# angela000/DQNFlappyBird

Hardware: NVIDIA B200
Metric: env frames/sec (step+render+preproc) (higher is better)
Workload: dtype u8

## Files before the change

dqnflappybird_b200/_lib.py:

```python
from __future__ import annotations

import ctypes as C
import glob
import os
import subprocess

_PKG = os.path.dirname(os.path.abspath(__file__))
_CSRC = os.path.join(_PKG, "csrc")
SO_PATH = os.path.join(_PKG, "libflappy_b200.so")

NVCC_FLAGS = [
    "-gencode", "arch=compute_100a,code=sm_100a", "-lineinfo", "-O3", "-std=c++17",
    "-Xcompiler", "-fPIC", "-shared",
]


class FlappyError(RuntimeError):
    pass


def sources():
    return sorted(glob.glob(os.path.join(_CSRC, "*.cu")))


# ... 61 lines not shown
                ("eps", C.c_float), ("grad_scale", C.c_float), ("beta1_power", C.c_float), ("beta2_power", C.c_float)]


_SIGNATURES = {
    "fb_last_error": ([], C.c_char_p),
    "fb_version": ([], C.c_int),
    "fb_assets_load": ([C.c_char_p, C.c_size_t], C.c_int),
    "fb_resize_tables": ([_i32p], C.c_int),
    "fb_env_create": ([C.c_int, C.c_uint64, C.c_uint64, C.POINTER(C.c_void_p)], C.c_int),
    "fb_env_destroy": ([_vp], C.c_int),
    "fb_env_num_envs": ([_vp], C.c_int),
    "fb_env_set_gap_replay": ([_vp, _u8p, C.c_int], C.c_int),
    "fb_env_reset": ([_vp, _vp], C.c_int),
    "fb_env_step": ([_vp, C.c_int, _u8p, _u8p, C.c_int, C.c_int, _f32p, _u8p, _i32p, _vp], C.c_int),
    "fb_env_draw": ([_vp, _u8p, C.c_int, C.c_int, _vp], C.c_int),
    "fb_env_step_random": ([_vp, C.c_int, C.c_uint64, C.c_uint32, C.c_uint32, _u8p, _u8p, C.c_int, C.c_int,
                            _f32p, _u8p, _i32p, _vp], C.c_int),
    "fb_env_step_host": ([_vp, _u8p, _u8p, C.c_int, C.c_int, _f32p, _u8p, _i32p, _vp], C.c_int),
    "fb_env_step_host_submit": ([_vp, _u8p, _u8p, C.c_int, C.c_int, _f32p, _u8p, _i32p, _vp], C.c_int),
    "fb_env_step_host_wait": ([_vp], C.c_int),
    "fb_env_check": ([_vp, _vp], C.c_int),
    "fb_env_export_state": ([_vp, _i32p, _vp], C.c_int),
    "fb_env_import_state": ([_vp, _i32p, _vp], C.c_int),
    "fb_env_obs_exact": ([_vp, _u8p, _vp], C.c_int),
    "fb_render_full": ([_vp, C.c_int, C.c_int, _u8p, _vp], C.c_int),
    "fb_log_episodes": ([_u8p, _i32p, C.c_int, C.c_int, C.c_int, _i32p, _i32p, C.c_int, _vp], C.c_int),
    "fb_qnet_create": ([C.c_int, C.c_int, C.c_int, C.POINTER(C.c_void_p)], C.c_int),
    "fb_qnet_destroy": ([_vp], C.c_int),
    "fb_qnet_set_precision": ([_vp, C.c_int], C.c_int),
    "fb_qnet_get_precision": ([_vp], C.c_int),
    "fb_qnet_invalidate": ([_vp], C.c_int),
    "fb_qnet_set_per_broadcast": ([_vp, C.c_int], C.c_int),
    "fb_debug_poison_packed": ([_vp, C.c_int, _vp], C.c_int),
    "fb_debug_write_probe": ([_vp, C.c_int, C.c_longlong, C.c_int, C.c_int, _vp], C.c_int),
    "fb_qnet_use_graphs": ([_vp, C.c_int], C.c_int),
    "fb_qnet_set_conv1_mode": ([_vp, C.c_int], C.c_int),
    "fb_qnet_set_fused_backward": ([_vp, C.c_int], C.c_int),
    "fb_qnet_param_count": ([_vp], C.c_int),
    "fb_qnet_layout": ([_vp, _i32p], C.c_int),
    "fb_qnet_forward": ([_vp, _f32p, _u8p, C.c_longlong, _i32p, C.c_int, _f32p, _vp], C.c_int),
    "fb_qnet_act": ([_vp, _f32p, _u8p, C.c_longlong, _i32p, C.c_int, C.c_double, C.c_uint64, C.c_uint64, _vp, _f32p, _u8p, _vp], C.c_int),
    "fb_qnet_adam": ([_vp, _f32p, _f32p, _f32p, _f32p, C.c_float, C.c_float, C.c_float, C.c_float, C.c_float, _vp], C.c_int),
    "fb_qnet_step": ([_vp, _vp, _vp], C.c_int),
    "fb_qnet_sync_target": ([_vp, _f32p, _f32p, _vp], C.c_int),
    "fb_noisy_layout": ([_vp, _i32p], C.c_int),
    "fb_noisy_draw": ([_vp, C.c_uint64, C.c_int, C.c_uint64, _f32p, _vp], C.c_int),
    "fb_noisy_weights": ([_vp, _f32p, _f32p, _f32p, _f32p, _vp], C.c_int),
    "fb_qnet_noisy_adam": ([_vp, _f32p, _f32p, _f32p, _f32p, _f32p, _f32p, _f32p, _f32p, C.c_float, C.c_float, C.c_float, C.c_float,
                            C.c_float, _vp], C.c_int),
    "fb_debug_struct_layout": ([C.c_int, _i32p, C.c_int], C.c_int),
    "fb_debug_step_sampling_layout": ([_i32p, C.c_int], C.c_int),
    "fb_dist_debug_stamps": ([_vp, _vp], C.c_int),
    "fb_dist_create": ([C.c_int, C.c_int, C.c_longlong, C.POINTER(C.c_void_p)], C.c_int),
    "fb_dist_destroy": ([_vp], C.c_int),
    "fb_dist_handle_bytes": ([], C.c_int),
    "fb_dist_set_two_shot": ([_vp, C.c_int], C.c_int),
    "fb_dist_debug_mask": ([_vp, C.c_int], C.c_int),
    "fb_dist_handles": ([_vp, C.c_char_p], C.c_int),
    "fb_dist_connect": ([_vp, C.c_char_p], C.c_int),
    "fb_dist_connect_local": ([_vp, C.c_int, _vp], C.c_int),
    "fb_dist_grads": ([_vp, C.c_int, C.POINTER(C.c_void_p)], C.c_int),
    "fb_dist_parity": ([_vp], C.c_int),
    "fb_dist_advance": ([_vp], C.c_int),
    "fb_qnet_attach_exchange": ([_vp, _vp], C.c_int),
    "fb_dist_adam": ([_vp, _vp, _f32p, _f32p, _f32p, C.c_float, C.c_float, C.c_float, C.c_float, C.c_float, _f32p, C.c_int, _vp], C.c_int),
    "fb_replay_create": ([C.c_int, C.c_int, C.c_int, C.c_int, C.c_int, C.POINTER(C.c_void_p)], C.c_int),
    "fb_replay_destroy": ([_vp], C.c_int),
# ... 61 lines not shown
```

dqnflappybird_b200/csrc/fb_debug.cu:

```cuda
#include <stddef.h>
#include <string.h>

#include "fb_env_logic.cuh"

extern "C" int fb_debug_host_step(int32_t *state16, int action, const uint8_t *gaps, int gaps_len, uint64_t seed,
                                  uint64_t env_id, float *reward, uint8_t *terminal, int32_t *score) {
    const ExactTables *ex = fb_host_exact_tables();
    if (!ex) { fb_set_error("fb_debug_host_step: load the assets first"); return FB_ERR_ASSETS; }
    FB_REQUIRE(state16 && reward && terminal && score, "fb_debug_host_step: NULL argument");
    if (action != 0 && action != 1) { fb_set_error("Multiple input actions!"); return FB_ERR_ACTION; }
    EnvState s;
    memset(&s, 0, sizeof(s));
    if (!ints_to_state(state16, s)) { fb_set_error("fb_debug_host_step: state outside the reachable range"); return FB_ERR_STATE; }
    GapSource g{gaps, gaps_len, seed, env_id};
    env_step(s, action, g, ex, *reward, *terminal, *score);
    state_to_ints(s, state16);
    return FB_OK;
}

extern "C" int fb_debug_host_reset(int32_t *state16, const uint8_t *gaps, int gaps_len, uint64_t seed, uint64_t env_id) {
    FB_REQUIRE(state16 != nullptr, "fb_debug_host_reset: NULL argument");
    EnvState s;
    memset(&s, 0, sizeof(s));
    GapSource g{gaps, gaps_len, seed, env_id};
// ... 35 lines not shown
    memset(&s, 0, sizeof(s));
    if (!ints_to_state(state16, s)) return -1;
    return (make_draw_list(s).np_mixed & 16) ? 1 : 0;
}

#define FB_OFF(S, f) (int32_t) offsetof(S, f)
extern "C" int fb_debug_struct_layout(int which, int32_t *out, int capacity) {
    typedef fb_step_sampling S;
    typedef fb_qnet_step_args A;
    const int32_t sampling[] = {(int32_t)sizeof(S), FB_OFF(S, replay), FB_OFF(S, ring_dev), FB_OFF(S, act_dev), FB_OFF(S, rew_dev),
                                FB_OFF(S, term_dev), FB_OFF(S, t), FB_OFF(S, batch), FB_OFF(S, setsize), FB_OFF(S, seed),
                                FB_OFF(S, idx_out_dev), FB_OFF(S, frames_out_dev), FB_OFF(S, act_out_dev), FB_OFF(S, rew_out_dev),
                                FB_OFF(S, term_out_dev), FB_OFF(S, env_out_dev), FB_OFF(S, k_out_dev), FB_OFF(S, prioritized),
                                FB_OFF(S, per_mode), FB_OFF(S, beta), FB_OFF(S, tree_idx_out_dev), FB_OFF(S, is_weights_out_dev),
                                FB_OFF(S, prio_out_dev), FB_OFF(S, is_weights_f32_out_dev), FB_OFF(S, n_step), FB_OFF(S, ret_out_dev),
                                FB_OFF(S, disc_out_dev)};
    const int32_t step[] = {(int32_t)sizeof(A), FB_OFF(A, variant), FB_OFF(A, loss_sum), FB_OFF(A, batch), FB_OFF(A, global_batch),
                            FB_OFF(A, gamma), FB_OFF(A, params_dev), FB_OFF(A, target_params_dev), FB_OFF(A, sampling),
                            FB_OFF(A, frames_dev), FB_OFF(A, sample_stride), FB_OFF(A, chan_off_s), FB_OFF(A, chan_off_next),
                            FB_OFF(A, actions_dev), FB_OFF(A, rewards_dev), FB_OFF(A, terminals_dev), FB_OFF(A, is_weights_dev),
                            FB_OFF(A, grads_dev), FB_OFF(A, loss_out_dev), FB_OFF(A, abs_err_out_dev), FB_OFF(A, q_target_out_dev),
                            FB_OFF(A, m_dev), FB_OFF(A, v_dev), FB_OFF(A, lr), FB_OFF(A, beta1), FB_OFF(A, beta2), FB_OFF(A, eps),
                            FB_OFF(A, grad_scale), FB_OFF(A, beta1_power), FB_OFF(A, beta2_power)};
    FB_REQUIRE(which == 0 || which == 1, "fb_debug_struct_layout: which must be 0 (fb_step_sampling) or 1 (fb_qnet_step_args)");
    const int32_t *v = which == 0 ? sampling : step;
    const int n = which == 0 ? (int)(sizeof(sampling) / sizeof(sampling[0])) : (int)(sizeof(step) / sizeof(step[0]));
    FB_REQUIRE(out != nullptr && capacity >= n, "fb_debug_struct_layout: buffer too small");
    for (int i = 0; i < n; i++) out[i] = v[i];
    return n;
}
#undef FB_OFF
extern "C" int fb_debug_step_sampling_layout(int32_t *out, int capacity) { return fb_debug_struct_layout(0, out, capacity); }

__global__ void __launch_bounds__(256) write_probe_kernel(uint8_t *dst, int n_chunks, long long stride_bytes, int mode) {
    extern __shared__ __align__(128) uint8_t stage_all[];
    const int warp = threadIdx.x >> 5, lane = threadIdx.x & 31;
    uint8_t *stage = stage_all + warp * 6400;
    const long long W = (long long)gridDim.x * 8, w = (long long)blockIdx.x * 8 + warp;
    const int lo = (int)((long long)n_chunks * w / W), hi = (int)((long long)n_chunks * (w + 1) / W);
    if (mode == 1) {
        for (int i = lane; i < 400; i += 32) reinterpret_cast<uint4 *>(stage)[i] = make_uint4(i, lane, 0xFFFFFFFFu, 0);
        asm volatile("fence.proxy.async.shared::cta;" ::: "memory");
        __syncwarp();
    }
    for (int k = lo; k < hi; k++) {
        uint8_t *out = dst + (long long)k * stride_bytes;
        if (mode == 0) {
            const uint4 v = make_uint4(k, lane, 0xFFFFFFFFu, 0);
#pragma unroll
            for (int it = 0; it < 13; it++) { int c = lane + 32 * it; if (c < 400) __stcs(reinterpret_cast<uint4 *>(out) + c, v); }
        } else if (lane == 0) {
            asm volatile("cp.async.bulk.wait_group.read 0;" ::: "memory");
            asm volatile("cp.async.bulk.global.shared::cta.bulk_group [%0], [%1], 6400;" ::"l"(reinterpret_cast<uint64_t>(out)),
                         "r"((uint32_t)__cvta_generic_to_shared(stage)) : "memory");
            asm volatile("cp.async.bulk.commit_group;" ::: "memory");
        }
    }
    if (mode == 1 && lane == 0) asm volatile("cp.async.bulk.wait_group 0;" ::: "memory");
}

extern "C" int fb_debug_write_probe(uint8_t *dst_dev, int n_chunks, long long stride_bytes, int mode, int ctas, void *stream) {
    FB_REQUIRE(dst_dev && n_chunks > 0 && stride_bytes >= 6400 && (mode == 0 || mode == 1) && ctas > 0, "fb_debug_write_probe: bad argument");
    FB_CUDA_OK(cudaFuncSetAttribute(write_probe_kernel, cudaFuncAttributeMaxDynamicSharedMemorySize, 8 * 6400));
    write_probe_kernel<<<ctas, 256, 8 * 6400, (cudaStream_t)stream>>>(dst_dev, n_chunks, stride_bytes, mode);
    FB_CUDA_OK(cudaGetLastError());
    return FB_OK;
}
```

dqnflappybird_b200/csrc/fb_env.cu:

```cuda
#include <stdlib.h>

#include <new>

#include "fb_env_logic.cuh"

struct fb_env {
    int n;
    uint64_t seed, first_id;
    EnvState *state;
    const uint8_t *gaps;
    int gaps_len;
    int *err_flag;
    uint8_t *stage_act[2];
    float *stage_rew[2];
    uint8_t *stage_term[2];
    int32_t *stage_score[2];
    cudaStream_t s_in, s_out;
    cudaEvent_t ev_in[2], ev_step[2], ev_out[2];
    unsigned long long submitted, waited;
    int num_sms;
    int step_slots;
};

struct StepArgs {
    EnvState *state;
    int n;
    uint64_t seed, first_id;
    const uint8_t *gaps;
    int gaps_len;
    const uint8_t *actions;
    uint64_t act_seed;
    uint32_t first_step, flap_threshold;
    uint8_t *actions_out;
    uint8_t *ring;
    int ring_len, ring_slot;
    float *reward;
    uint8_t *terminal;
    int32_t *score;
    int n_steps;
    int draw_only;
    int *err_flag;
    const ObsTables *obs_tab;
    const ExactTables *ex;
};

__device__ __forceinline__ uint32_t expand4(uint32_t nib) {
    return ((nib * 0x00204081u) & 0x01010101u) * 255u;
}

struct RowConst { int sx[3], tab[3]; };

struct __align__(16) DrawWords {
    int px[3];
    int flags;
    int goff[3];
    int bird;
};
__device__ __forceinline__ DrawWords to_words(const ObsTables &T, const DrawList &d) {
    DrawWords w;
    const int np = d.np_mixed & 15;
#pragma unroll
    for (int k = 0; k < 3; k++) { w.px[k] = k < np ? (int)d.px[k] : 9999; w.goff[k] = (int)d.gap[k] * 8; }
    w.flags = ((d.np_mixed & 16) ? 1 : 0) | ((int)T.birdJ0[d.y] << 1) | ((int)d.y << 8) | ((int)d.pidx << 20) | (np << 24);
    w.bird = ((int)d.pidx * (kMaxY + 1) + (int)d.y) * (kBirdRows + 3);
    return w;
}

constexpr int kChunks = kObs * 5;

__device__ __forceinline__ void render_env(const ObsTables &T, const uint2 *lut8, const ExactTables *ex, const DrawWords w,
                                           const RowConst &rc, unsigned short *m16, unsigned long long *fixrows, uint8_t *out, int lane) {
    const int j0 = (w.flags >> 1) & 127;
    const unsigned char *pipe_bytes = reinterpret_cast<const unsigned char *>(&T.pipeObs[0][0][0]);
    const unsigned char *bird_bytes = reinterpret_cast<const unsigned char *>(&T.birdObs[0][0][0]) + w.bird;
// ... 21 lines not shown
            int idx = q * 32 + lane, r = idx >> 3, j = j0 + (idx & 7);
            int bit = 0;
            if (r < kBirdRows && j < kBaseJ) bit = exact_obs_bit(ex, d, 0, false, 16 + r, j);
            unsigned bal = __ballot_sync(0xFFFFFFFFu, bit);
            int rr = 4 * q + lane;
            if (lane < 4 && rr < kBirdRows) fixrows[rr] = obs_row_fix(fixrows[rr], (bal >> (8 * lane)) & 0xFFu, j0);
        }
        __syncwarp();
        if (lane >= 16 && lane < 16 + kBirdRows) m[0] = fixrows[lane - 16];
    }
#pragma unroll
    for (int it = 0; it < 3; it++) {
        const int i = lane + 32 * it;
        if (i < kObs) {
            unsigned short *row = m16 + 5 * i;
            row[0] = (unsigned short)m[it]; row[1] = (unsigned short)(m[it] >> 16);
            row[2] = (unsigned short)(m[it] >> 32); row[3] = (unsigned short)(m[it] >> 48);
        }
    }
    __syncwarp();
    const unsigned short *mine = m16 + lane;
    uint4 *dst = reinterpret_cast<uint4 *>(out) + lane;
#pragma unroll
    for (int it = 0; it < 13; it++) {
        if (it < 12 || lane < kChunks - 32 * 12) {
            const uint32_t bits = mine[32 * it];
            const uint2 a = lut8[bits & 255u], b = lut8[bits >> 8];
            __stcs(dst + 32 * it, make_uint4(a.x, a.y, b.x, b.y));
        }
    }
    __syncwarp();
}

constexpr int kStepThreads = 256, kStepWarps = kStepThreads / 32;

__global__ void __launch_bounds__(kStepThreads, 4) env_step_kernel(const StepArgs a) {
    extern __shared__ __align__(16) unsigned char t_raw[];
    ObsTables &T = *reinterpret_cast<ObsTables *>(t_raw);
    __shared__ __align__(16) HitTables H;
    __shared__ DrawWords dw[kStepWarps][32];
    __shared__ __align__(16) unsigned short m16[kStepWarps][kChunks + 8];
    __shared__ unsigned long long fixrows[kStepWarps][kBirdRows + 1];
    __shared__ uint2 lut8[256];
    const int tid = threadIdx.x, warp = tid >> 5, lane = tid & 31;
    asm volatile("griddepcontrol.launch_dependents;");
    lut8[tid] = make_uint2(expand4(tid & 15u), expand4(tid >> 4));

    {
        const uint4 *srcH = reinterpret_cast<const uint4 *>(a.ex);
        uint4 *dstH = reinterpret_cast<uint4 *>(&H);
        for (int k = tid; k < (int)(sizeof(HitTables) / 16); k += kStepThreads) dstH[k] = __ldg(srcH + k);
    }
    if (a.ring) {
        const uint4 *src = reinterpret_cast<const uint4 *>(a.obs_tab);
        uint4 *dstT = reinterpret_cast<uint4 *>(&T);
        for (int k = tid; k < (int)(sizeof(ObsTables) / 16); k += kStepThreads) dstT[k] = __ldg(src + k);
    }
    __syncthreads();
    asm volatile("griddepcontrol.wait;" ::: "memory");

    RowConst rc;
#pragma unroll
    for (int it = 0; it < 3; it++) {
        const int i = min(lane + 32 * it, kObs - 1);
        rc.sx[it] = T.sx[i]; rc.tab[it] = (i - 5 * ((i * 205) >> 10)) * 64;
    }
    for (int i = lane; i < kObs; i += 32) m16[warp][5 * i + 4] = 0xFFFFu;
    __syncwarp();
    const long long W = (long long)gridDim.x * kStepWarps, w = (long long)blockIdx.x * kStepWarps + warp;
    const int lo = (int)((long long)a.n * w / W), hi = (int)((long long)a.n * (w + 1) / W);
    for (int base = lo; base < hi; base += 32) {
        const int e_mine = base + lane;
        const bool have = e_mine < hi;
        const int n_here = min(32, hi - base);
        EnvState s;
        GapSource gs;
        if (have) {
            const uint4 *sp = reinterpret_cast<const uint4 *>(a.state + e_mine);
            uint4 v0 = sp[0], v1 = sp[1];
            *reinterpret_cast<uint4 *>(&s) = v0;
            *(reinterpret_cast<uint4 *>(&s) + 1) = v1;
            gs.script = a.gaps ? a.gaps + (size_t)e_mine * a.gaps_len : nullptr;
            gs.script_len = a.gaps_len;
            gs.seed = a.seed; gs.env_id = a.first_id + (uint64_t)e_mine;
        }
        for (int step = 0; step < a.n_steps; step++) {
            if (have && a.draw_only) dw[warp][lane] = to_words(T, make_draw_list(s));
            if (have && !a.draw_only) {
                int act;
                const size_t o = (size_t)step * a.n + e_mine;
                if (a.actions) {
                    act = a.actions[o];
                    if (act > 1) { atomicOr(a.err_flag, 1); act = 0; }
                } else {
                    act = stream_word(a.act_seed, 1u, gs.env_id, a.first_step + (uint32_t)step) < a.flap_threshold ? 1 : 0;
                    if (a.actions_out) a.actions_out[o] = (uint8_t)act;
                }
                float rew; uint8_t term; int32_t sc;
                env_step(s, act, gs, &H, rew, term, sc);
                if (a.reward) a.reward[o] = rew;
                if (a.terminal) a.terminal[o] = term;
                if (a.score) a.score[o] = sc;
                if (a.ring) dw[warp][lane] = to_words(T, make_draw_list(s));
            }
            if (a.ring) {
                const int slot = (a.ring_slot + step) % a.ring_len;
                __syncwarp();
                for (int e = 0; e < n_here; e++) {
                    uint8_t *out = a.ring + ((size_t)(base + e) * a.ring_len + slot) * (size_t)FB_FRAME_BYTES;
                    render_env(T, lut8, a.ex, dw[warp][e], rc, m16[warp], fixrows[warp], out, lane);
                }
                __syncwarp();
            }
        }
        if (have) {
            uint4 *sp = reinterpret_cast<uint4 *>(a.state + e_mine);
            sp[0] = *reinterpret_cast<uint4 *>(&s);
            sp[1] = *(reinterpret_cast<uint4 *>(&s) + 1);
        }
    }
}


__global__ void env_reset_kernel(EnvState *state, int n, uint64_t seed, uint64_t first_id, const uint8_t *gaps, int gaps_len) {
    int e = blockIdx.x * blockDim.x + threadIdx.x;
    if (e >= n) return;
    EnvState s;
    memset(&s, 0, sizeof(s));
    GapSource gs{gaps ? gaps + (size_t)e * gaps_len : nullptr, gaps_len, seed, first_id + (uint64_t)e};
    env_reset(s, gs);
    state[e] = s;
}

__global__ void env_export_kernel(const EnvState *state, int n, int32_t *out) {
    int e = blockIdx.x * blockDim.x + threadIdx.x;
    if (e >= n) return;
    EnvState s = state[e];
    state_to_ints(s, out + (size_t)e * FB_STATE_INTS);
}

__global__ void env_import_kernel(EnvState *state, int n, const int32_t *in, int *err_flag) {
    int e = blockIdx.x * blockDim.x + threadIdx.x;
    if (e >= n) return;
    EnvState s;
    if (!ints_to_state(in + (size_t)e * FB_STATE_INTS, s)) { atomicOr(err_flag, 2); return; }
    state[e] = s;
}

__global__ void env_obs_exact_kernel(const EnvState *state, int n, const ExactTables *ex, uint8_t *obs) {
    int e = blockIdx.x;
    if (e >= n) return;
    __shared__ DrawList d;
// ... 5 lines not shown
        obs[(size_t)e * FB_FRAME_BYTES + p] = exact_obs_bit(ex, d, basex, true, i, j) ? 255 : 0;
    }
}

__global__ void env_render_full_kernel(const EnvState *state, int first, int n, const ExactTables *ex, uint8_t *rgb) {
    int e = blockIdx.y;
    if (e >= n) return;
    __shared__ DrawList d;
    __shared__ int basex;
    if (threadIdx.x == 0) { EnvState s = state[first + e]; d = make_draw_list(s); basex = s.basex; }
    __syncthreads();
    int p = blockIdx.x * blockDim.x + threadIdx.x;
    if (p >= kScreenW * kScreenH) return;
    int X = p / kScreenH, Y = p - X * kScreenH;
    uint32_t c = scene_rgb(ex, d, basex, true, X, Y);
    uint8_t *o = rgb + ((size_t)e * kScreenW * kScreenH + p) * 3;
    o[0] = c & 255; o[1] = (c >> 8) & 255; o[2] = (c >> 16) & 255;
}


extern "C" int fb_env_create(int n_envs, uint64_t seed, uint64_t first_env_id, fb_env **out) {
    FB_REQUIRE(out != nullptr, "fb_env_create: out is NULL");
    FB_REQUIRE(n_envs > 0, "fb_env_create: n_envs must be positive");
    if (!fb_tables().loaded) { fb_set_error("fb_env_create: call fb_assets_load first"); return FB_ERR_ASSETS; }
    fb_env *e = new (std::nothrow) fb_env();
    FB_REQUIRE(e != nullptr, "fb_env_create: out of host memory");
    e->n = n_envs; e->seed = seed; e->first_id = first_env_id; e->gaps = nullptr; e->gaps_len = 0;
    int dev = 0;
    FB_CUDA_OK(cudaGetDevice(&dev));
    FB_CUDA_OK(cudaDeviceGetAttribute(&e->num_sms, cudaDevAttrMultiProcessorCount, dev));
    FB_CUDA_OK(cudaMalloc(&e->state, sizeof(EnvState) * (size_t)n_envs));
    FB_CUDA_OK(cudaMalloc(&e->err_flag, sizeof(int)));
    FB_CUDA_OK(cudaMemset(e->err_flag, 0, sizeof(int)));
    for (int k = 0; k < 2; k++) {
        FB_CUDA_OK(cudaMalloc(&e->stage_act[k], (size_t)n_envs));
        FB_CUDA_OK(cudaMalloc(&e->stage_rew[k], sizeof(float) * (size_t)n_envs));
        FB_CUDA_OK(cudaMalloc(&e->stage_term[k], (size_t)n_envs));
        FB_CUDA_OK(cudaMalloc(&e->stage_score[k], sizeof(int32_t) * (size_t)n_envs));
        FB_CUDA_OK(cudaEventCreateWithFlags(&e->ev_in[k], cudaEventDisableTiming));
        FB_CUDA_OK(cudaEventCreateWithFlags(&e->ev_step[k], cudaEventDisableTiming));
        FB_CUDA_OK(cudaEventCreateWithFlags(&e->ev_out[k], cudaEventDisableTiming));
    }
    FB_CUDA_OK(cudaStreamCreateWithFlags(&e->s_in, cudaStreamNonBlocking));
    FB_CUDA_OK(cudaStreamCreateWithFlags(&e->s_out, cudaStreamNonBlocking));
    e->submitted = e->waited = 0;
    e->step_slots = 0;
    *out = e;
    return fb_env_reset(e, nullptr);
}

extern "C" int fb_env_destroy(fb_env *e) {
    if (!e) return FB_OK;
    cudaFree(e->state); cudaFree(e->err_flag);
    for (int k = 0; k < 2; k++) {
        cudaFree(e->stage_act[k]); cudaFree(e->stage_rew[k]); cudaFree(e->stage_term[k]); cudaFree(e->stage_score[k]);
        if (e->ev_in[k]) cudaEventDestroy(e->ev_in[k]);
        if (e->ev_step[k]) cudaEventDestroy(e->ev_step[k]);
        if (e->ev_out[k]) cudaEventDestroy(e->ev_out[k]);
    }
    if (e->s_in) cudaStreamDestroy(e->s_in);
    if (e->s_out) cudaStreamDestroy(e->s_out);
    delete e;
    return FB_OK;
}

extern "C" int fb_env_num_envs(const fb_env *e) { return e ? e->n : 0; }

extern "C" int fb_env_set_gap_replay(fb_env *e, const uint8_t *gaps_dev, int per_env_len) {
    FB_REQUIRE(e != nullptr, "fb_env_set_gap_replay: env is NULL");
    FB_REQUIRE(gaps_dev == nullptr || per_env_len > 0, "fb_env_set_gap_replay: per_env_len must be positive");
    e->gaps = gaps_dev; e->gaps_len = gaps_dev ? per_env_len : 0;
    return FB_OK;
}

extern "C" int fb_env_reset(fb_env *e, void *stream) {
    FB_REQUIRE(e != nullptr, "fb_env_reset: env is NULL");
    env_reset_kernel<<<(e->n + 255) / 256, 256, 0, (cudaStream_t)stream>>>(e->state, e->n, e->seed, e->first_id, e->gaps, e->gaps_len);
    FB_CUDA_OK(cudaGetLastError());
    return FB_OK;
}

static int launch_step(fb_env *e, StepArgs &a, cudaStream_t st, bool early = true) {
    a.state = e->state; a.n = e->n; a.seed = e->seed; a.first_id = e->first_id;
    a.gaps = e->gaps; a.gaps_len = e->gaps_len; a.err_flag = e->err_flag;
    a.obs_tab = fb_tables().obs_dev; a.ex = fb_tables().exact_dev;
    if (e->step_slots == 0) {
        FB_CUDA_OK(cudaFuncSetAttribute(env_step_kernel, cudaFuncAttributeMaxDynamicSharedMemorySize, (int)sizeof(ObsTables)));
        int per_sm = 0;
        FB_CUDA_OK(cudaOccupancyMaxActiveBlocksPerMultiprocessor(&per_sm, env_step_kernel, kStepThreads, sizeof(ObsTables)));
        FB_REQUIRE(per_sm >= 1, "env_step_kernel does not fit an SM");
        e->step_slots = per_sm * e->num_sms;
    }
    static int oversub = 0;
    if (oversub == 0) { const char *v = getenv("FB_ENV_OVERSUB"); oversub = (v && v[0] >= '1' && v[0] <= '8') ? v[0] - '0' : 1; }
    long long warps = (long long)e->step_slots * kStepWarps * oversub;
    if (warps > e->n) warps = e->n;
    const int grid = (int)((warps + kStepWarps - 1) / kStepWarps);
    cudaLaunchConfig_t cfg{};
    cfg.gridDim = dim3(grid); cfg.blockDim = dim3(kStepThreads); cfg.dynamicSmemBytes = sizeof(ObsTables); cfg.stream = st;
    cudaLaunchAttribute at[1];
    at[0].id = cudaLaunchAttributeProgrammaticStreamSerialization;
    static int pdl = -1;
    if (pdl < 0) { const char *v = getenv("FB_ENV_PDL"); pdl = (v && v[0] == '0') ? 0 : 1; }
    at[0].val.programmaticStreamSerializationAllowed = pdl && early ? 1 : 0;
    cfg.attrs = at; cfg.numAttrs = 1;
    FB_CUDA_OK(cudaLaunchKernelEx(&cfg, env_step_kernel, (const StepArgs)a));
    return FB_OK;
}

static int check_ring(const fb_env *e, const uint8_t *ring, int ring_len, int ring_slot, int n_steps) {
    FB_REQUIRE(e != nullptr, "fb_env_step: env is NULL");
    FB_REQUIRE(n_steps > 0, "fb_env_step: n_steps must be positive");
    if (ring) {
        FB_REQUIRE(ring_len > 0 && ring_slot >= 0 && ring_slot < ring_len, "fb_env_step: ring_slot outside the ring");
        FB_REQUIRE((reinterpret_cast<uintptr_t>(ring) & 15) == 0, "fb_env_step: obs ring must be 16-byte aligned");
    }
    return FB_OK;
}

extern "C" int fb_env_step(fb_env *e, int n_steps, const uint8_t *actions_dev, uint8_t *obs_ring_dev, int ring_len,
                           int ring_slot, float *reward_dev, uint8_t *terminal_dev, int32_t *score_dev, void *stream) {
    int rc = check_ring(e, obs_ring_dev, ring_len, ring_slot, n_steps);
    if (rc) return rc;
    FB_REQUIRE(actions_dev != nullptr, "fb_env_step: actions_dev is NULL");
    StepArgs a{};
    a.actions = actions_dev; a.ring = obs_ring_dev; a.ring_len = ring_len; a.ring_slot = ring_slot;
    a.reward = reward_dev; a.terminal = terminal_dev; a.score = score_dev; a.n_steps = n_steps;
    return launch_step(e, a, (cudaStream_t)stream);
}

extern "C" int fb_env_draw(fb_env *e, uint8_t *obs_ring_dev, int ring_len, int ring_slot, void *stream) {
    int rc = check_ring(e, obs_ring_dev, ring_len, ring_slot, 1);
    if (rc) return rc;
    FB_REQUIRE(obs_ring_dev != nullptr, "fb_env_draw: obs_ring_dev is NULL");
    StepArgs a{};
    a.ring = obs_ring_dev; a.ring_len = ring_len; a.ring_slot = ring_slot; a.n_steps = 1; a.draw_only = 1;
    return launch_step(e, a, (cudaStream_t)stream);
}

// ... 122 lines not shown
```

include/flappy_b200.h:

```cpp
#ifndef FLAPPY_B200_H
#define FLAPPY_B200_H

#include <stddef.h>
#include <stdint.h>

#ifdef __cplusplus
extern "C" {
#endif

#define FB_OBS 80
#define FB_FRAME_BYTES 6400
#define FB_SCREEN_W 288
#define FB_SCREEN_H 512
#define FB_STATE_INTS 16

typedef enum {
    FB_OK = 0,
    FB_ERR_INVALID = -1,
    FB_ERR_CUDA = -2,
    FB_ERR_ASSETS = -3,
    FB_ERR_ACTION = -4,
    FB_ERR_STATE = -5
} fb_status;

// ... 20 lines not shown
int fb_env_step_random(fb_env *env, int n_steps, uint64_t action_seed, uint32_t first_step, uint32_t flap_threshold,
                       uint8_t *actions_out_dev, uint8_t *obs_ring_dev, int ring_len, int ring_slot,
                       float *reward_dev, uint8_t *terminal_dev, int32_t *score_dev, void *stream);

int fb_env_step_host(fb_env *env, const uint8_t *actions_host, uint8_t *obs_ring_dev, int ring_len, int ring_slot,
                     float *reward_host, uint8_t *terminal_host, int32_t *score_host, void *stream);
int fb_env_step_host_submit(fb_env *env, const uint8_t *actions_host, uint8_t *obs_ring_dev, int ring_len, int ring_slot,
                            float *reward_host, uint8_t *terminal_host, int32_t *score_host, void *stream);
int fb_env_step_host_wait(fb_env *env);

int fb_env_check(fb_env *env, void *stream);

int fb_env_export_state(fb_env *env, int32_t *out_dev, void *stream);
int fb_env_import_state(fb_env *env, const int32_t *in_dev, void *stream);

int fb_env_obs_exact(fb_env *env, uint8_t *obs_dev, void *stream);

int fb_render_full(fb_env *env, int first, int n, uint8_t *rgb_dev, void *stream);

int fb_resize_tables(int32_t *out_host);

typedef struct fb_qnet fb_qnet;
int fb_qnet_create(int hidden, int dueling, int max_batch, fb_qnet **out);
int fb_qnet_destroy(fb_qnet *net);

#define FB_PRECISION_FP32 0
#define FB_PRECISION_BF16 1
#define FB_PRECISION_FP16 2
int fb_qnet_set_precision(fb_qnet *net, int precision);
int fb_qnet_get_precision(const fb_qnet *net);
int fb_qnet_invalidate(fb_qnet *net);
int fb_qnet_set_per_broadcast(fb_qnet *net, int on);
int fb_debug_poison_packed(fb_qnet *net, int slot, void *stream);
int fb_debug_write_probe(uint8_t *dst_dev, int n_chunks, long long stride_bytes, int mode, int ctas, void *stream);
int fb_qnet_use_graphs(fb_qnet *net, int enable);
int fb_qnet_set_conv1_mode(fb_qnet *net, int mode);
int fb_qnet_set_fused_backward(fb_qnet *net, int on);
int fb_qnet_param_count(const fb_qnet *net);
int fb_qnet_layout(const fb_qnet *net, int32_t *out16_host);

int fb_qnet_forward(fb_qnet *net, const float *params_dev, const uint8_t *frames_dev, long long sample_stride,
                    const int32_t *chan_off_host4, int batch, float *q_out_dev, void *stream);

int fb_qnet_act(fb_qnet *net, const float *params_dev, const uint8_t *frames_dev, long long sample_stride,
                const int32_t *chan_off_host4, int batch, double epsilon, uint64_t seed, uint64_t first_env_id,
                uint32_t *rng_pos_dev, float *q_out_dev, uint8_t *actions_out_dev, void *stream);

int fb_qnet_adam(fb_qnet *net, float *params_dev, const float *grads_dev, float *m_dev, float *v_dev, float alpha,
                 float beta1, float beta2, float eps, float grad_scale, void *stream);

int fb_qnet_sync_target(fb_qnet *net, float *target_dev, const float *params_dev, void *stream);

int fb_noisy_layout(const fb_qnet *net, int32_t *out20_host);
int fb_noisy_draw(fb_qnet *net, uint64_t seed, int role, uint64_t counter, float *factors_dev, void *stream);
int fb_noisy_weights(fb_qnet *net, const float *mu_dev, const float *sigma_dev, const float *factors_dev, float *weff_dev, void *stream);
int fb_qnet_noisy_adam(fb_qnet *net, float *mu_dev, float *sigma_dev, const float *grads_dev, const float *factors_dev, float *m_dev,
                       float *v_dev, float *sigma_m_dev, float *sigma_v_dev, float alpha, float beta1, float beta2, float eps,
                       float grad_scale, void *stream);

typedef struct fb_dist fb_dist;
int fb_dist_create(int rank, int world, long long n_floats, fb_dist **out);
int fb_dist_destroy(fb_dist *d);
int fb_dist_handle_bytes(void);
int fb_dist_set_two_shot(fb_dist *d, int on);
int fb_dist_handles(fb_dist *d, uint8_t *out_host);
int fb_dist_connect(fb_dist *d, const uint8_t *all_handles_host);
int fb_dist_connect_local(fb_dist *d, int q, fb_dist *peer);
// ... 83 lines not shown
```

Baseline: 835.0 million.

## Split env step into producer physics warps and consumer render warps via mbarrier queues

The fused step kernel is restructured so that 4 physics warps per CTA grab batches of 32 envs from a global atomic counter, step them, and push draw lists into per-warp shared-memory queues guarded by mbarriers. 20 drawing warps pull individual env frames from those queues and render them. This replaces the static per-warp env partition in which each warp alternated between physics and serial rendering of 32 frames. Physics-only calls (no ring) now go to a separate lighter kernel without the obs tables. The write-probe debug kernel gains ordering and residency options. The change adds atomics, barrier overhead and a self-resetting global counter, which could race across overlapping launches.

```diff
diff --git a/dqnflappybird_b200/_lib.py b/dqnflappybird_b200/_lib.py
--- a/dqnflappybird_b200/_lib.py
+++ b/dqnflappybird_b200/_lib.py
@@ -117,7 +117,7 @@
     "fb_qnet_invalidate": ([_vp], C.c_int),
     "fb_qnet_set_per_broadcast": ([_vp, C.c_int], C.c_int),
     "fb_debug_poison_packed": ([_vp, C.c_int, _vp], C.c_int),
-    "fb_debug_write_probe": ([_vp, C.c_int, C.c_longlong, C.c_int, C.c_int, _vp], C.c_int),
+    "fb_debug_write_probe": ([_vp, C.c_int, C.c_longlong, C.c_int, C.c_int, C.c_int, C.c_int, _vp], C.c_int),
     "fb_qnet_use_graphs": ([_vp, C.c_int], C.c_int),
     "fb_qnet_set_conv1_mode": ([_vp, C.c_int], C.c_int),
     "fb_qnet_set_fused_backward": ([_vp, C.c_int], C.c_int),
diff --git a/dqnflappybird_b200/csrc/fb_debug.cu b/dqnflappybird_b200/csrc/fb_debug.cu
--- a/dqnflappybird_b200/csrc/fb_debug.cu
+++ b/dqnflappybird_b200/csrc/fb_debug.cu
@@ -91,21 +91,24 @@
 #undef FB_OFF
 extern "C" int fb_debug_step_sampling_layout(int32_t *out, int capacity) { return fb_debug_struct_layout(0, out, capacity); }
 
-__global__ void __launch_bounds__(256) write_probe_kernel(uint8_t *dst, int n_chunks, long long stride_bytes, int mode) {
+__device__ unsigned int g_probe_next, g_probe_done;
+
+__global__ void __launch_bounds__(256) write_probe_kernel(uint8_t *dst, int n_chunks, long long stride_bytes, int mode, int order) {
     extern __shared__ __align__(128) uint8_t stage_all[];
     const int warp = threadIdx.x >> 5, lane = threadIdx.x & 31;
     uint8_t *stage = stage_all + warp * 6400;
     const long long W = (long long)gridDim.x * 8, w = (long long)blockIdx.x * 8 + warp;
-    const int lo = (int)((long long)n_chunks * w / W), hi = (int)((long long)n_chunks * (w + 1) / W);
     if (mode == 1) {
         for (int i = lane; i < 400; i += 32) reinterpret_cast<uint4 *>(stage)[i] = make_uint4(i, lane, 0xFFFFFFFFu, 0);
         asm volatile("fence.proxy.async.shared::cta;" ::: "memory");
         __syncwarp();
     }
-    for (int k = lo; k < hi; k++) {
-        uint8_t *out = dst + (long long)k * stride_bytes;
+    long long k = order == 0 ? n_chunks * w / W : w, hi = order == 0 ? n_chunks * (w + 1) / W : n_chunks;
+    if (order == 2) k = __shfl_sync(0xFFFFFFFFu, lane == 0 ? atomicAdd(&g_probe_next, 1u) : 0u, 0);
+    while (k < hi) {
+        uint8_t *out = dst + k * stride_bytes;
         if (mode == 0) {
-            const uint4 v = make_uint4(k, lane, 0xFFFFFFFFu, 0);
+            const uint4 v = make_uint4((uint32_t)k, lane, 0xFFFFFFFFu, 0);
 #pragma unroll
             for (int it = 0; it < 13; it++) { int c = lane + 32 * it; if (c < 400) __stcs(reinterpret_cast<uint4 *>(out) + c, v); }
         } else if (lane == 0) {
@@ -114,14 +117,30 @@
                          "r"((uint32_t)__cvta_generic_to_shared(stage)) : "memory");
             asm volatile("cp.async.bulk.commit_group;" ::: "memory");
         }
+        if (order == 0) k++;
+        else if (order == 1) k += W;
+        else k = __shfl_sync(0xFFFFFFFFu, lane == 0 ? atomicAdd(&g_probe_next, 1u) : 0u, 0);
     }
     if (mode == 1 && lane == 0) asm volatile("cp.async.bulk.wait_group 0;" ::: "memory");
+    if (order == 2) {
+        __syncthreads();
+        if (threadIdx.x == 0 && atomicAdd(&g_probe_done, 1u) == gridDim.x - 1) { g_probe_next = 0; g_probe_done = 0; __threadfence(); }
+    }
 }
 
-extern "C" int fb_debug_write_probe(uint8_t *dst_dev, int n_chunks, long long stride_bytes, int mode, int ctas, void *stream) {
-    FB_REQUIRE(dst_dev && n_chunks > 0 && stride_bytes >= 6400 && (mode == 0 || mode == 1) && ctas > 0, "fb_debug_write_probe: bad argument");
-    FB_CUDA_OK(cudaFuncSetAttribute(write_probe_kernel, cudaFuncAttributeMaxDynamicSharedMemorySize, 8 * 6400));
-    write_probe_kernel<<<ctas, 256, 8 * 6400, (cudaStream_t)stream>>>(dst_dev, n_chunks, stride_bytes, mode);
+extern "C" int fb_debug_write_probe(uint8_t *dst_dev, int n_chunks, long long stride_bytes, int mode, int order, int ctas_per_sm,
+                                    int ctas, void *stream) {
+    FB_REQUIRE(dst_dev && n_chunks > 0 && stride_bytes >= 6400 && (mode == 0 || mode == 1) && order >= 0 && order <= 2 &&
+               ctas_per_sm >= 1 && ctas_per_sm <= 8 && ctas > 0, "fb_debug_write_probe: bad argument");
+    int dev = 0, smem_sm = 0, per_sm = 0;
+    FB_CUDA_OK(cudaGetDevice(&dev));
+    FB_CUDA_OK(cudaDeviceGetAttribute(&smem_sm, cudaDevAttrMaxSharedMemoryPerMultiprocessor, dev));
+    const int smem = ((smem_sm / ctas_per_sm - 1024) / 128) * 128;
+    FB_REQUIRE(mode == 0 || smem >= 8 * 6400, "fb_debug_write_probe: mode 1 stages 51,200 bytes a CTA: at most 4 CTAs per SM");
+    FB_CUDA_OK(cudaFuncSetAttribute(write_probe_kernel, cudaFuncAttributeMaxDynamicSharedMemorySize, smem));
+    FB_CUDA_OK(cudaOccupancyMaxActiveBlocksPerMultiprocessor(&per_sm, write_probe_kernel, 256, smem));
+    FB_REQUIRE(per_sm == ctas_per_sm, "fb_debug_write_probe: could not set the residency");
+    write_probe_kernel<<<ctas, 256, smem, (cudaStream_t)stream>>>(dst_dev, n_chunks, stride_bytes, mode, order);
     FB_CUDA_OK(cudaGetLastError());
     return FB_OK;
 }
diff --git a/dqnflappybird_b200/csrc/fb_env.cu b/dqnflappybird_b200/csrc/fb_env.cu
--- a/dqnflappybird_b200/csrc/fb_env.cu
+++ b/dqnflappybird_b200/csrc/fb_env.cu
@@ -3,6 +3,7 @@
 #include <new>
 
 #include "fb_env_logic.cuh"
+#include "fb_tc.cuh"
 
 struct fb_env {
     int n;
@@ -19,7 +20,8 @@
     cudaEvent_t ev_in[2], ev_step[2], ev_out[2];
     unsigned long long submitted, waited;
     int num_sms;
-    int step_slots;
+    int step_slots, phys_slots;
+    unsigned *batch_ctr;
 };
 
 struct StepArgs {
@@ -40,6 +42,7 @@
     int n_steps;
     int draw_only;
     int *err_flag;
+    unsigned *batch_ctr;
     const ObsTables *obs_tab;
     const ExactTables *ex;
 };
@@ -127,92 +130,155 @@
     __syncwarp();
 }
 
-constexpr int kStepThreads = 256, kStepWarps = kStepThreads / 32;
-
-__global__ void __launch_bounds__(kStepThreads, 4) env_step_kernel(const StepArgs a) {
+__device__ __forceinline__ void physics_step(const StepArgs &a, EnvState &s, const GapSource &gs, const HitTables *H, int e, int step) {
+    int act;
+    const size_t o = (size_t)step * a.n + e;
+    if (a.actions) {
+        act = a.actions[o];
+        if (act > 1) { atomicOr(a.err_flag, 1); act = 0; }
+    } else {
+        act = stream_word(a.act_seed, 1u, gs.env_id, a.first_step + (uint32_t)step) < a.flap_threshold ? 1 : 0;
+        if (a.actions_out) a.actions_out[o] = (uint8_t)act;
+    }
+    float rew; uint8_t term; int32_t sc;
+    env_step(s, act, gs, H, rew, term, sc);
+    if (a.reward) a.reward[o] = rew;
+    if (a.terminal) a.terminal[o] = term;
+    if (a.score) a.score[o] = sc;
+}
+
+__device__ __forceinline__ void load_env(const StepArgs &a, int e, EnvState &s, GapSource &gs) {
+    const uint4 *sp = reinterpret_cast<const uint4 *>(a.state + e);
+    *reinterpret_cast<uint4 *>(&s) = sp[0];
+    *(reinterpret_cast<uint4 *>(&s) + 1) = sp[1];
+    gs.script = a.gaps ? a.gaps + (size_t)e * a.gaps_len : nullptr;
+    gs.script_len = a.gaps_len;
+    gs.seed = a.seed; gs.env_id = a.first_id + (uint64_t)e;
+}
+
+__device__ __forceinline__ void store_env(const StepArgs &a, int e, const EnvState &s) {
+    uint4 *sp = reinterpret_cast<uint4 *>(a.state + e);
+    sp[0] = *reinterpret_cast<const uint4 *>(&s);
+    sp[1] = *(reinterpret_cast<const uint4 *>(&s) + 1);
+}
+
+__device__ __forceinline__ void load_hit_tables(const StepArgs &a, HitTables &H, int tid, int threads) {
+    const uint4 *src = reinterpret_cast<const uint4 *>(a.ex);
+    uint4 *dst = reinterpret_cast<uint4 *>(&H);
+    for (int k = tid; k < (int)(sizeof(HitTables) / 16); k += threads) dst[k] = __ldg(src + k);
+}
+
+constexpr int kPhysThreads = 256;
+
+__global__ void __launch_bounds__(kPhysThreads, 4) env_physics_kernel(const StepArgs a) {
+    __shared__ __align__(16) HitTables H;
+    asm volatile("griddepcontrol.launch_dependents;");
+    load_hit_tables(a, H, threadIdx.x, kPhysThreads);
+    __syncthreads();
+    asm volatile("griddepcontrol.wait;" ::: "memory");
+    for (int e = blockIdx.x * kPhysThreads + threadIdx.x; e < a.n; e += gridDim.x * kPhysThreads) {
+        EnvState s;
+        GapSource gs;
+        load_env(a, e, s, gs);
+        for (int step = 0; step < a.n_steps; step++) physics_step(a, s, gs, &H, e, step);
+        store_env(a, e, s);
+    }
+}
+
+constexpr int kPhysWarps = 4, kDrawWarps = 20, kStepThreads = 32 * (kPhysWarps + kDrawWarps), kStepCtasPerSm = 2, kQueue = 4;
+static_assert(kDrawWarps % kPhysWarps == 0 && kDrawWarps / kPhysWarps <= 32, "every queue has the same number of drawing warps, at most 32");
+
+struct __align__(16) DrawItem {
+    DrawList d[32];
+    int base, slot, count, pad;
+};
+
+__global__ void __launch_bounds__(kStepThreads, kStepCtasPerSm) env_step_kernel(const StepArgs a) {
     extern __shared__ __align__(16) unsigned char t_raw[];
     ObsTables &T = *reinterpret_cast<ObsTables *>(t_raw);
     __shared__ __align__(16) HitTables H;
-    __shared__ DrawWords dw[kStepWarps][32];
-    __shared__ __align__(16) unsigned short m16[kStepWarps][kChunks + 8];
-    __shared__ unsigned long long fixrows[kStepWarps][kBirdRows + 1];
+    __shared__ DrawItem queue[kPhysWarps][kQueue];
+    __shared__ __align__(8) uint64_t full[kPhysWarps][kQueue], empty[kPhysWarps][kQueue];
+    __shared__ __align__(16) unsigned short m16[kDrawWarps][kChunks + 8];
+    __shared__ unsigned long long fixrows[kDrawWarps][kBirdRows + 1];
     __shared__ uint2 lut8[256];
+    __shared__ int next_job[kPhysWarps];
     const int tid = threadIdx.x, warp = tid >> 5, lane = tid & 31;
     asm volatile("griddepcontrol.launch_dependents;");
-    lut8[tid] = make_uint2(expand4(tid & 15u), expand4(tid >> 4));
-
+    for (int k = tid; k < 256; k += kStepThreads) lut8[k] = make_uint2(expand4(k & 15u), expand4(k >> 4));
+    if (!a.draw_only) load_hit_tables(a, H, tid, kStepThreads);
     {
-        const uint4 *srcH = reinterpret_cast<const uint4 *>(a.ex);
-        uint4 *dstH = reinterpret_cast<uint4 *>(&H);
-        for (int k = tid; k < (int)(sizeof(HitTables) / 16); k += kStepThreads) dstH[k] = __ldg(srcH + k);
-    }
-    if (a.ring) {
         const uint4 *src = reinterpret_cast<const uint4 *>(a.obs_tab);
         uint4 *dstT = reinterpret_cast<uint4 *>(&T);
         for (int k = tid; k < (int)(sizeof(ObsTables) / 16); k += kStepThreads) dstT[k] = __ldg(src + k);
     }
+    if (tid < kPhysWarps) {
+        for (int k = 0; k < kQueue; k++) { tc::mbar_init(tc::smem_u32(&full[tid][k]), 32); tc::mbar_init(tc::smem_u32(&empty[tid][k]), 32); }
+        next_job[tid] = 0;
+        tc::fence_barrier_init();
+    }
     __syncthreads();
     asm volatile("griddepcontrol.wait;" ::: "memory");
 
+    if (warp < kPhysWarps) {
+        DrawItem *q = queue[warp];
+        int item = 0;
+        for (;;) {
+            int b = 0;
+            if (lane == 0) b = (int)atomicAdd(a.batch_ctr, 1u);
+            const int base = __shfl_sync(0xFFFFFFFFu, b, 0) * 32;
+            if (base >= a.n) break;
+            const int e = base + lane;
+            const bool have = e < a.n;
+            EnvState s;
+            GapSource gs;
+            if (have) load_env(a, e, s, gs);
+            for (int step = 0; step < a.n_steps; step++) {
+                if (have && !a.draw_only) physics_step(a, s, gs, &H, e, step);
+                const int qs = item % kQueue;
+                if (item >= kQueue) tc::mbar_wait(tc::smem_u32(&empty[warp][qs]), (item / kQueue - 1) & 1);
+                if (have) q[qs].d[lane] = make_draw_list(s);
+                if (lane == 0) { q[qs].base = base; q[qs].slot = (a.ring_slot + step) % a.ring_len; q[qs].count = min(32, a.n - base); }
+                tc::mbar_arrive(tc::smem_u32(&full[warp][qs]));
+                item++;
+            }
+            if (have && !a.draw_only) store_env(a, e, s);
+        }
+        const int qs = item % kQueue;
+        if (item >= kQueue) tc::mbar_wait(tc::smem_u32(&empty[warp][qs]), (item / kQueue - 1) & 1);
+        if (lane == 0) q[qs].count = -1;
+        tc::mbar_arrive(tc::smem_u32(&full[warp][qs]));
+        if (lane == 0) {
+            __threadfence();
+            if (atomicAdd(a.batch_ctr + 1, 1u) == gridDim.x * kPhysWarps - 1) { atomicExch(a.batch_ctr, 0u); atomicExch(a.batch_ctr + 1, 0u); }
+        }
+        return;
+    }
+    const int dw = warp - kPhysWarps, p = dw % kPhysWarps;
+    const DrawItem *q = queue[p];
     RowConst rc;
 #pragma unroll
     for (int it = 0; it < 3; it++) {
         const int i = min(lane + 32 * it, kObs - 1);
         rc.sx[it] = T.sx[i]; rc.tab[it] = (i - 5 * ((i * 205) >> 10)) * 64;
     }
-    for (int i = lane; i < kObs; i += 32) m16[warp][5 * i + 4] = 0xFFFFu;
+    for (int i = lane; i < kObs; i += 32) m16[dw][5 * i + 4] = 0xFFFFu;
     __syncwarp();
-    const long long W = (long long)gridDim.x * kStepWarps, w = (long long)blockIdx.x * kStepWarps + warp;
-    const int lo = (int)((long long)a.n * w / W), hi = (int)((long long)a.n * (w + 1) / W);
-    for (int base = lo; base < hi; base += 32) {
-        const int e_mine = base + lane;
-        const bool have = e_mine < hi;
-        const int n_here = min(32, hi - base);
-        EnvState s;
-        GapSource gs;
-        if (have) {
-            const uint4 *sp = reinterpret_cast<const uint4 *>(a.state + e_mine);
-            uint4 v0 = sp[0], v1 = sp[1];
-            *reinterpret_cast<uint4 *>(&s) = v0;
-            *(reinterpret_cast<uint4 *>(&s) + 1) = v1;
-            gs.script = a.gaps ? a.gaps + (size_t)e_mine * a.gaps_len : nullptr;
-            gs.script_len = a.gaps_len;
-            gs.seed = a.seed; gs.env_id = a.first_id + (uint64_t)e_mine;
-        }
-        for (int step = 0; step < a.n_steps; step++) {
-            if (have && a.draw_only) dw[warp][lane] = to_words(T, make_draw_list(s));
-            if (have && !a.draw_only) {
-                int act;
-                const size_t o = (size_t)step * a.n + e_mine;
-                if (a.actions) {
-                    act = a.actions[o];
-                    if (act > 1) { atomicOr(a.err_flag, 1); act = 0; }
-                } else {
-                    act = stream_word(a.act_seed, 1u, gs.env_id, a.first_step + (uint32_t)step) < a.flap_threshold ? 1 : 0;
-                    if (a.actions_out) a.actions_out[o] = (uint8_t)act;
-                }
-                float rew; uint8_t term; int32_t sc;
-                env_step(s, act, gs, &H, rew, term, sc);
-                if (a.reward) a.reward[o] = rew;
-                if (a.terminal) a.terminal[o] = term;
-                if (a.score) a.score[o] = sc;
-                if (a.ring) dw[warp][lane] = to_words(T, make_draw_list(s));
-            }
-            if (a.ring) {
-                const int slot = (a.ring_slot + step) % a.ring_len;
-                __syncwarp();
-                for (int e = 0; e < n_here; e++) {
-                    uint8_t *out = a.ring + ((size_t)(base + e) * a.ring_len + slot) * (size_t)FB_FRAME_BYTES;
-                    render_env(T, lut8, a.ex, dw[warp][e], rc, m16[warp], fixrows[warp], out, lane);
-                }
-                __syncwarp();
-            }
-        }
-        if (have) {
-            uint4 *sp = reinterpret_cast<uint4 *>(a.state + e_mine);
-            sp[0] = *reinterpret_cast<uint4 *>(&s);
-            sp[1] = *(reinterpret_cast<uint4 *>(&s) + 1);
-        }
+    for (;;) {
+        int j = 0;
+        if (lane == 0) j = atomicAdd(&next_job[p], 1);
+        j = __shfl_sync(0xFFFFFFFFu, j, 0);
+        const int item = j >> 5, e = j & 31, qs = item % kQueue;
+        tc::mbar_wait(tc::smem_u32(&full[p][qs]), (item / kQueue) & 1);
+        const int count = q[qs].count;
+        if (count < 0) break;
+        const bool draw = e < count;
+        DrawWords w;
+        size_t frame = 0;
+        if (draw) { w = to_words(T, q[qs].d[e]); frame = (size_t)(q[qs].base + e) * a.ring_len + q[qs].slot; }
+        __syncwarp();
+        if (lane == 0) tc::mbar_arrive(tc::smem_u32(&empty[p][qs]));
+        if (draw) render_env(T, lut8, a.ex, w, rc, m16[dw], fixrows[dw], a.ring + frame * FB_FRAME_BYTES, lane);
     }
 }
 
@@ -284,6 +350,8 @@
     FB_CUDA_OK(cudaMalloc(&e->state, sizeof(EnvState) * (size_t)n_envs));
     FB_CUDA_OK(cudaMalloc(&e->err_flag, sizeof(int)));
     FB_CUDA_OK(cudaMemset(e->err_flag, 0, sizeof(int)));
+    FB_CUDA_OK(cudaMalloc(&e->batch_ctr, 2 * sizeof(unsigned)));
+    FB_CUDA_OK(cudaMemset(e->batch_ctr, 0, 2 * sizeof(unsigned)));
     for (int k = 0; k < 2; k++) {
         FB_CUDA_OK(cudaMalloc(&e->stage_act[k], (size_t)n_envs));
         FB_CUDA_OK(cudaMalloc(&e->stage_rew[k], sizeof(float) * (size_t)n_envs));
@@ -296,14 +364,14 @@
     FB_CUDA_OK(cudaStreamCreateWithFlags(&e->s_in, cudaStreamNonBlocking));
     FB_CUDA_OK(cudaStreamCreateWithFlags(&e->s_out, cudaStreamNonBlocking));
     e->submitted = e->waited = 0;
-    e->step_slots = 0;
+    e->step_slots = e->phys_slots = 0;
     *out = e;
     return fb_env_reset(e, nullptr);
 }
 
 extern "C" int fb_env_destroy(fb_env *e) {
     if (!e) return FB_OK;
-    cudaFree(e->state); cudaFree(e->err_flag);
+    cudaFree(e->state); cudaFree(e->err_flag); cudaFree(e->batch_ctr);
     for (int k = 0; k < 2; k++) {
         cudaFree(e->stage_act[k]); cudaFree(e->stage_rew[k]); cudaFree(e->stage_term[k]); cudaFree(e->stage_score[k]);
         if (e->ev_in[k]) cudaEventDestroy(e->ev_in[k]);
@@ -334,7 +402,7 @@
 
 static int launch_step(fb_env *e, StepArgs &a, cudaStream_t st, bool early = true) {
     a.state = e->state; a.n = e->n; a.seed = e->seed; a.first_id = e->first_id;
-    a.gaps = e->gaps; a.gaps_len = e->gaps_len; a.err_flag = e->err_flag;
+    a.gaps = e->gaps; a.gaps_len = e->gaps_len; a.err_flag = e->err_flag; a.batch_ctr = e->batch_ctr;
     a.obs_tab = fb_tables().obs_dev; a.ex = fb_tables().exact_dev;
     if (e->step_slots == 0) {
         FB_CUDA_OK(cudaFuncSetAttribute(env_step_kernel, cudaFuncAttributeMaxDynamicSharedMemorySize, (int)sizeof(ObsTables)));
@@ -342,21 +410,24 @@
         FB_CUDA_OK(cudaOccupancyMaxActiveBlocksPerMultiprocessor(&per_sm, env_step_kernel, kStepThreads, sizeof(ObsTables)));
         FB_REQUIRE(per_sm >= 1, "env_step_kernel does not fit an SM");
         e->step_slots = per_sm * e->num_sms;
-    }
-    static int oversub = 0;
-    if (oversub == 0) { const char *v = getenv("FB_ENV_OVERSUB"); oversub = (v && v[0] >= '1' && v[0] <= '8') ? v[0] - '0' : 1; }
-    long long warps = (long long)e->step_slots * kStepWarps * oversub;
-    if (warps > e->n) warps = e->n;
-    const int grid = (int)((warps + kStepWarps - 1) / kStepWarps);
+        FB_CUDA_OK(cudaOccupancyMaxActiveBlocksPerMultiprocessor(&per_sm, env_physics_kernel, kPhysThreads, 0));
+        FB_REQUIRE(per_sm >= 1, "env_physics_kernel does not fit an SM");
+        e->phys_slots = per_sm * e->num_sms;
+    }
     cudaLaunchConfig_t cfg{};
-    cfg.gridDim = dim3(grid); cfg.blockDim = dim3(kStepThreads); cfg.dynamicSmemBytes = sizeof(ObsTables); cfg.stream = st;
+    if (a.ring) {
+        cfg.gridDim = dim3(min(e->step_slots, (e->n + 31) / 32)); cfg.blockDim = dim3(kStepThreads); cfg.dynamicSmemBytes = sizeof(ObsTables);
+    } else {
+        cfg.gridDim = dim3(min(e->phys_slots, (e->n + kPhysThreads - 1) / kPhysThreads)); cfg.blockDim = dim3(kPhysThreads);
+    }
+    cfg.stream = st;
     cudaLaunchAttribute at[1];
     at[0].id = cudaLaunchAttributeProgrammaticStreamSerialization;
     static int pdl = -1;
     if (pdl < 0) { const char *v = getenv("FB_ENV_PDL"); pdl = (v && v[0] == '0') ? 0 : 1; }
     at[0].val.programmaticStreamSerializationAllowed = pdl && early ? 1 : 0;
     cfg.attrs = at; cfg.numAttrs = 1;
-    FB_CUDA_OK(cudaLaunchKernelEx(&cfg, env_step_kernel, (const StepArgs)a));
+    FB_CUDA_OK(cudaLaunchKernelEx(&cfg, a.ring ? env_step_kernel : env_physics_kernel, (const StepArgs)a));
     return FB_OK;
 }
 
diff --git a/include/flappy_b200.h b/include/flappy_b200.h
--- a/include/flappy_b200.h
+++ b/include/flappy_b200.h
@@ -76,7 +76,8 @@
 int fb_qnet_invalidate(fb_qnet *net);
 int fb_qnet_set_per_broadcast(fb_qnet *net, int on);
 int fb_debug_poison_packed(fb_qnet *net, int slot, void *stream);
-int fb_debug_write_probe(uint8_t *dst_dev, int n_chunks, long long stride_bytes, int mode, int ctas, void *stream);
+int fb_debug_write_probe(uint8_t *dst_dev, int n_chunks, long long stride_bytes, int mode, int order, int ctas_per_sm, int ctas,
+                         void *stream);
 int fb_qnet_use_graphs(fb_qnet *net, int enable);
 int fb_qnet_set_conv1_mode(fb_qnet *net, int mode);
 int fb_qnet_set_fused_backward(fb_qnet *net, int on);
```

Result: faster. 894.7 million, median of 6 (+7.1%).
